# populationgenomics/cuKING

Hardware: AMD Instinct MI355X
Metric: sample-pairs/s (all-pairs KING) (higher is better)
Workload: dtype fp4 products, f32 accumulate (exact integers)

## Files before the change

cuking_amd/csrc/king_abi.hip:

```cpp
#include <hip/hip_runtime.h>

#include <algorithm>
#include <cstdio>
#include <cstdlib>
#include <cstring>
#include <vector>

#include "king_common.h"
#include "king_host.h"
#include "king_kin_summary.h"

using namespace cuking;

namespace {

#define HIP_TRY(expr)                                                      \
  do {                                                                     \
    const hipError_t _e = (expr);                                          \
    if (_e != hipSuccess) {                                                \
      (void)hipGetLastError();  \
      return cuking_fail(_e == hipErrorOutOfMemory ? CUKING_ERR_OUT_OF_MEMORY     \
                                            : CUKING_ERR_DEVICE,           \
                  "%s failed: %s", #expr, hipGetErrorString(_e));          \
    }                                                                      \
// ... 68 lines not shown
  struct StreamScratch {
    hipStream_t stream;
    uint32_t *split = nullptr;
    uint8_t *filter = nullptr;
    uint64_t filter_tiles = 0;
  };
  std::vector<StreamScratch> scratch;
  unsigned long long filter_totals_retired[kNumTotals] = {};
  uint32_t filter_quadrant_cap = kFilterQuadrantCap;
  uint32_t filter_cand_cap = kFilterCandCap;
  uint32_t filter_split_min_steps = 8;
  int filter_check0 = 1, filter_check1 = 1, filter_check_emit = (int)kCheckEmitCap;
  int filter_rotate = 1;
  uint32_t filter_rotate_min_steps = 128;
  uint32_t filter_rotate_min_tiles = 2048;
  int filter_sort = 1;
  bool filter_lazy_codes = true;
  void *sort_temp = nullptr;
  size_t sort_temp_bytes = 0;

  void *synth_tables = nullptr;
  size_t synth_tables_bytes = 0;
  hipStream_t synth_stream = nullptr;
  hipEvent_t synth_done = nullptr;

  struct Prepared {
    bool valid = false;
    cuking_submatrix sm = {0, 0, 0, 0};
    uint32_t words_per_sample = 0;
    int variant = -1;
// ... 179 lines not shown
         kin_threshold > 0.f && kin_threshold < 0.5f;
}

LaunchSwitches launch_switches(const cuking_ctx *ctx, uint32_t words_per_sample, bool full,
                               float kin_threshold) {
  LaunchSwitches sw;
  sw.xcd_swizzle = (uint32_t)ctx->xcd_swizzle;
  sw.dyn_tail_tiles = ctx->dyn_tail_tiles;
  sw.check0 = (uint32_t)ctx->filter_check0;
  sw.check1 = (uint32_t)ctx->filter_check1;
  sw.check_emit = (uint32_t)ctx->filter_check_emit;
  sw.rotate = (uint32_t)ctx->filter_rotate;
  sw.rotate_min_tiles = ctx->filter_rotate_min_tiles;
  sw.split_min_steps = ctx->filter_split_min_steps;
  sw.filter_runs = filter_runs(ctx, words_per_sample, full, kin_threshold);
  return sw;
}

struct Outputs {
  uint32_t max_results;
  cuking_result *results;
  uint32_t *result_index, *result_overflow;
  cuking_counts *counts;
  float *kin;
  uint64_t kin_ld;
  uint32_t kin_flags;
  uint64_t *sum_hist, *sum_best;
  cuking_kin_bins sum_bins;
  uint32_t *rel_counts;
  uint32_t rel_num;
// ... 32 lines not shown
  if (out.rel_counts != nullptr) {
    a.rel_num = out.rel_num;
    for (uint32_t t = 0; t < out.rel_num; ++t) a.rel_thr[t] = out.rel_thr[t];
  }
  a.rect_row_stride = 1;
  a.bits = d_bit_sets;
  a.words_per_sample = words_per_sample;
  a.split_wgs = ctx->split_wgs;
  if (plan_variant(ctx, words_per_sample).layout == kLayoutNibbleStats) {
    a.perm = plane_perm(ctx->planes, geo);
    if (!ctx->prepared.codes) a.codes_ready = plane_flags(ctx->planes, geo);
  }
  cuking_ctx::StreamScratch *e;
  const cuking_status st = scratch_for(ctx, stream, block_tiles, &e);
  if (st != CUKING_OK || e == nullptr) return st;
  if (uses_split_slab(ctx)) {
    a.split_counters = e->split;
    a.split_scratch = e->split + mfma_split_counter_bytes(ctx->split_wgs) / sizeof(uint32_t);
  }
  if (!uses_filter_scratch(ctx)) return CUKING_OK;
  uint8_t *base = e->filter;
  const FilterScratchLayout l = filter_scratch_layout(e->filter_tiles);
  a.sample_stats = plane_stats(ctx->planes, geo);
  a.t2 = plane_t2(ctx->planes, geo);
  a.prefix_u = plane_prefix_u(ctx->planes, geo);
  a.cohort_sums = plane_cohort_sums(ctx->planes, geo);
  a.filter_ctrl = reinterpret_cast<uint32_t *>(base);
  a.filter_totals = reinterpret_cast<unsigned long long *>(base + l.totals);
  a.fsplit_tickets = reinterpret_cast<uint32_t *>(base + l.tickets);
  a.tile_done = base + l.tile_done;
  a.cand_list = reinterpret_cast<uint2 *>(base + l.cand);
  a.cand_cap = ctx->filter_cand_cap < l.cand_entries ? ctx->filter_cand_cap : l.cand_entries;
  a.quadrant_cap = ctx->filter_quadrant_cap;
  a.dense_list = reinterpret_cast<uint2 *>(base + l.dense);
  a.dense_cap = l.chunk_tiles * 4;
  a.fsplit_slabs = ctx->split_wgs != 0 ? reinterpret_cast<float4 *>(base + l.slabs) : nullptr;
  a.rotate_min_steps = ctx->filter_rotate_min_steps;
  a.check_steps = plane_check_steps(ctx->planes, geo);
  return CUKING_OK;
}

hipError_t launch_planned(const cuking_ctx *ctx, uint32_t words_per_sample, bool full,
                          TiledArgs a, const LaunchSwitches &sw, uint64_t num_tiles,
                          hipStream_t stream) {
  const int kv = effective_variant(ctx, words_per_sample);
  if (tiled_variant(kv).tile != tiled_variant(ctx->variant).tile) {
    if (tiled_variant(kv).tile * 2 != tiled_variant(ctx->variant).tile) return hipErrorInvalidValue;
    to_quadrants(&a, &num_tiles);
  }
  return launch_tiled(kv, full, a, sw, num_tiles, stream);
}

// ... 312 lines not shown
    {"filter_sort", 0, 2, "filter_sort outside [0, 2]", 0, kInvalidatesLayout,
     CTX_FIELD(filter_sort)},
    {"filter_lazy_codes", 0, 1, "filter_lazy_codes outside [0, 1]", 0, kInvalidatesLayout,
     CTX_FIELD(filter_lazy_codes)},
    {"filter_check0", 0, 2, "filter_check0 outside [0, 2]", 0, 0, CTX_FIELD(filter_check0)},
    {"filter_check1", 0, 1 + kNumCheckShares, "filter_check1 outside {0, 1, 3 .. %u}",
     1 + kNumCheckShares, 0, CTX_FIELD(filter_check1), 2},
    {"filter_check_emit", 0, 255, "filter_check_emit outside [0, 255]", 0, 0,
     CTX_FIELD(filter_check_emit)},
    {"filter_rotate", 0, 2 + kNumPhases, "filter_rotate outside [0, %u]", 2 + kNumPhases, 0,
     CTX_FIELD(filter_rotate)},
    {"filter_rotate_min_steps", 1, 1 << 20, "filter_rotate_min_steps outside [1, 2^20]", 0, 0,
     CTX_FIELD(filter_rotate_min_steps)},
    {"filter_rotate_min_tiles", 0, 1 << 30, "filter_rotate_min_tiles outside [0, 2^30]", 0, 0,
     CTX_FIELD(filter_rotate_min_tiles)},
    {"filter_quadrant_cap", 0, 16384, "filter_quadrant_cap outside [0, 16384]", 0, 0,
     CTX_FIELD(filter_quadrant_cap)},
    {"filter_cand_cap", 0, kFilterCandCap, "filter_cand_cap outside [0, %u]", kFilterCandCap, 0,
     CTX_FIELD(filter_cand_cap)},
    {"filter_split_min_steps", 1, 4096, "filter_split_min_steps outside [1, 4096]", 0, 0,
     CTX_FIELD(filter_split_min_steps)},
    {"max_launch_blocks", 0, INT64_MAX, "negative block cap", 0, 0,
     [](const cuking_ctx *) -> int64_t { return (int64_t)max_blocks_override(); },
     [](cuking_ctx *, int64_t v) { set_max_blocks_per_launch((uint64_t)v); }},
    {"filter_check_min_steps", 4, 1 << 20, "filter_check_min_steps outside [4, 2^20]", 0,
     kInvalidatesLayout,
     [](const cuking_ctx *) -> int64_t { return filter_check_min_steps(); },
     [](cuking_ctx *, int64_t v) { set_filter_check_min_steps((uint32_t)v); }},
};
#undef CTX_FIELD
// ... 930 lines not shown
```

cuking_amd/csrc/king_common.h:

```cpp
#ifndef CUKING_AMD_KING_COMMON_H_
#define CUKING_AMD_KING_COMMON_H_

#include <hip/hip_runtime.h>
#include <stdint.h>

#include "cuking_amd.h"
#include "king_launch_plan.h"
#include "king_submatrix.h"

namespace cuking {

constexpr uint32_t kLayoutWord = 0;
constexpr uint32_t kLayoutQuad = 1;
constexpr uint32_t kLayoutNibble = 2;
constexpr uint32_t kLayoutNibbleStats = 3;

struct PlaneGeometry {
  uint32_t num_rows, num_cols;
  uint32_t rows_padded, cols_padded;
  uint32_t col_base;
  uint32_t s_stride;
  uint32_t k_words;
  uint32_t diag;
};
// ... 87 lines not shown
  const uint32_t *gate;
  uint32_t gate_count;
  const uint8_t *skip_tiles;
  uint64_t skip_base;
  const uint32_t *perm;
  uint32_t *codes_ready;
  float *dense_kin;
  uint64_t kin_ld;
  uint32_t kin_diag;
  unsigned long long *sum_hist, *sum_best;
  float sum_lo, sum_scale;
  uint32_t sum_bins;
  uint32_t *rel_counts;
  uint32_t rel_num;
  float rel_thr[CUKING_REL_THRESHOLDS_MAX];
};

constexpr uint32_t kCheckEmitCap = 64;
constexpr uint32_t kNumCheckShares = 8;
constexpr uint32_t kCheckShares64[kNumCheckShares] = {8, 50, 53, 56, 58, 60, 61, 62};
constexpr uint32_t kNumPhases = 128;
constexpr uint32_t kPhasesPerShare = kNumPhases / 64;
constexpr uint32_t kNumCum = kNumPhases - 1;
__host__ __device__ inline uint32_t phase_step(uint32_t all_steps, uint32_t x) {
  return (uint32_t)((uint64_t)all_steps * x / kNumPhases);
}
__host__ __device__ inline uint32_t check_step_of(uint32_t all_steps, uint32_t k,
                                                  uint32_t min_steps = 64) {
  if (all_steps < min_steps) return 0;
  return phase_step(all_steps, kCheckShares64[k] * kPhasesPerShare);
}
constexpr uint32_t kFilterSplitSlabs = 256;
constexpr size_t kFilterSlabBytes = 256 * 256 * sizeof(float);
constexpr size_t kFilterTicketBytes = kFilterSplitSlabs * sizeof(uint32_t);
__host__ __device__ inline size_t plane_bytes(const PlaneGeometry &g,
                                              uint32_t layout) {
  const size_t base = (size_t)g.k_words * g.s_stride * (layout == kLayoutQuad ? 8 : 16);
  if (layout == kLayoutNibble) return base + base / 4;
  if (layout == kLayoutNibbleStats)
    return base + base / 4 + base / 2 + (size_t)g.s_stride * sizeof(float2) +
// ... 34 lines not shown
static_assert(4ull * kMfmaN4MaxSites <= (1ull << 24), "filter kernel: exact float sums");
constexpr int kMfmaN4Stages = 5;
constexpr uint32_t kMfmaN4LdsBytes = kMfmaN4Stages * 2 * 2 * 4 * 128 * 16;
static_assert(kMfmaN4LdsBytes <= 160 * 1024, "LDS of one CU");
constexpr int kMfmaFilterVariant = 7;
constexpr uint32_t kFilterTile = 256;
constexpr uint32_t kFilterLdsBytes = 5 * 2 * 2 * 2 * 256 * 16;
static_assert(kFilterLdsBytes <= 160 * 1024, "LDS of one CU");
constexpr uint32_t kFilterChunkTiles = 1u << 17;
constexpr uint32_t kFilterCandCap = 1u << 25;
constexpr uint32_t kFilterQuadrantCap = 384;
constexpr size_t kFilterCtrlBytes = 256;
constexpr uint32_t kCtrlCand = 0, kCtrlDense = 1, kCtrlDyn = 2, kCtrlFinished = 3,
                   kCtrlLeft = 4, kCtrlAllLeave = 5, kCtrlGate = 6;
constexpr uint32_t kCtrlStepTicks = 8, kCtrlPos = 16, kPosSlots = 16;
constexpr size_t kCtrlChunkBytes = (kCtrlPos + 8 * kPosSlots * 2) * 4;
constexpr uint32_t kTotalCand = 0, kTotalDense = 1, kTotalEarly = 2, kTotalRotated = 3;
constexpr uint32_t kNumTotals = 4;
__host__ __device__ inline const uint32_t *plane_check_steps(const uint4 *planes,
                                                             const PlaneGeometry &g) {
  return reinterpret_cast<const uint32_t *>(plane_cohort_sums(planes, g) + 8);
}
__host__ __device__ inline uint32_t *plane_flags(const uint4 *planes, const PlaneGeometry &g) {
  return const_cast<uint32_t *>(plane_check_steps(planes, g)) + 16;
}
__host__ __device__ inline uint32_t *plane_perm(const uint4 *planes, const PlaneGeometry &g) {
  return plane_flags(planes, g) + 16;
}
__host__ __device__ inline float2 *plane_tmp_stats(const uint4 *planes, const PlaneGeometry &g) {
  return reinterpret_cast<float2 *>(plane_perm(planes, g) + g.s_stride);
}
// ... 32 lines not shown
constexpr uint32_t kMfmaLdsBytes = kMfmaStages * 2 * 2 * 2 * 128 * 16;
constexpr uint32_t kMfmaParkBytes = 4 * 64 * 64 * 4;
static_assert(kMfmaLdsBytes + kMfmaParkBytes <= 160 * 1024, "LDS of one CU");
const TiledVariant &tiled_variant(int v);
hipError_t launch_tiled(int variant, bool full, const TiledArgs &args, const LaunchSwitches &sw,
                        uint64_t num_tiles, hipStream_t stream);
hipError_t launch_mfma(bool full, bool nibble, const TiledArgs &args, const LaunchSwitches &sw,
                       uint64_t num_tiles, uint32_t lds_bytes, hipStream_t stream);
hipError_t launch_mfma_kin(bool nibble, const TiledArgs &args, const LaunchSwitches &sw,
                           uint64_t num_tiles, hipStream_t stream);
hipError_t launch_mfma_summary(bool nibble, const TiledArgs &args, const LaunchSwitches &sw,
                               uint64_t num_tiles, hipStream_t stream);
hipError_t launch_kin_mirror(float *d_kin, uint64_t ld, uint32_t n, hipStream_t stream);
hipError_t launch_mfma_list(const TiledArgs &args, const uint2 *list, const uint32_t *count,
                            uint32_t cap, uint32_t grid, hipStream_t stream);
hipError_t launch_mfma_gated(const TiledArgs &args, uint64_t num_units, const uint32_t *gate,
                             const uint8_t *skip_tiles, uint64_t skip_base, uint32_t grid,
                             hipStream_t stream);
hipError_t launch_filter(const TiledArgs &args, const LaunchSwitches &sw, uint64_t num_tiles,
                         hipStream_t stream);
inline void to_quadrants(TiledArgs *a, uint64_t *num_units) {
  a->quad = 1;
  a->tile_begin *= 4;
  *num_units *= 4;
}
hipError_t launch_sample_stats(const uint64_t *d_bit_sets, uint32_t words_per_sample,
                               const PlaneGeometry &geo, uint4 *d_planes, uint32_t s_begin,
                               uint32_t s_end, hipStream_t stream);
void set_filter_check_min_steps(uint32_t steps);
uint32_t filter_check_min_steps();
size_t sort_temp_bytes_for(uint32_t n);
hipError_t launch_sample_order(const PlaneGeometry &geo, uint32_t words_per_sample,
                               uint4 *d_planes, uint32_t s_begin, uint32_t s_end, bool sort,
                               void *sort_temp, size_t sort_temp_bytes, hipStream_t stream);
hipError_t launch_prepare_nibbles(bool codes, bool t2, const uint64_t *d_bit_sets,
                                  uint32_t words_per_sample, const PlaneGeometry &geo,
                                  uint4 *d_planes, const uint32_t *perm, uint32_t s_tile_begin,
                                  uint32_t s_tile_end, const uint32_t *gate,
                                  const uint32_t *ready, hipStream_t stream);
hipError_t launch_mark_codes_ready(const uint32_t *gate, uint32_t *ready, hipStream_t stream);
size_t mfma_split_scratch_bytes(uint32_t wgs);
size_t mfma_split_counter_bytes(uint32_t wgs);

void set_max_blocks_per_launch(uint64_t blocks);
uint64_t max_blocks_override();

hipError_t launch_prepare_planes(uint32_t layout, const uint64_t *d_bit_sets,
                                 uint32_t words_per_sample,
                                 const PlaneGeometry &geo, uint4 *d_planes,
                                 uint32_t s_tile_begin, uint32_t s_tile_end,
                                 hipStream_t stream);

hipError_t launch_stream(const cuking_submatrix &sm, uint32_t words_per_sample,
                         const uint64_t *d_bit_sets, float kin_threshold,
                         uint32_t max_results, cuking_result *d_results,
                         uint32_t *d_result_index, uint32_t *d_result_overflow,
                         cuking_counts *d_dense_counts, float *d_dense_kin, uint64_t kin_ld,
// ... 29 lines not shown
```

cuking_amd/csrc/king_device.h:

```cpp
#ifndef CUKING_AMD_KING_DEVICE_H_
#define CUKING_AMD_KING_DEVICE_H_

#include <hip/hip_runtime.h>

#include <atomic>

#include "king_common.h"

namespace cuking {

typedef __attribute__((address_space(3))) void *lds_void_ptr;
typedef const __attribute__((address_space(1))) void *global_void_ptr;

template <typename T>
__device__ __forceinline__ T relaxed_load(const T *p) {
  return __hip_atomic_load(p, __ATOMIC_RELAXED, __HIP_MEMORY_SCOPE_AGENT);
}
template <typename T, typename V>
__device__ __forceinline__ void relaxed_store(T *p, V v) {
  __hip_atomic_store(p, (T)v, __ATOMIC_RELAXED, __HIP_MEMORY_SCOPE_AGENT);
}
template <typename T, typename V>
__device__ __forceinline__ T relaxed_add(T *p, V v) {
  return __hip_atomic_fetch_add(p, (T)v, __ATOMIC_RELAXED, __HIP_MEMORY_SCOPE_AGENT);
// ... 5 lines not shown
  uint32_t lane, wave;
  uint32_t wy, wx;
  uint32_t g, lr;
};
__device__ __forceinline__ Lanes lanes_of_thread() {
  const uint32_t lane = threadIdx.x & 63;
  const uint32_t wave = __builtin_amdgcn_readfirstlane(threadIdx.x >> 6);
  return Lanes{lane, wave, wave >> 1, wave & 1, lane >> 5, lane & 31};
}

__device__ __forceinline__ uint32_t c_row(int r, uint32_t g) { return (r & 3) + 8 * (r >> 2) + 4 * g; }

__device__ __forceinline__ uint32_t xcd_patch_tile(uint32_t wg) {
  const uint32_t x = wg & 7, j = wg >> 3;
  return (((j >> 5) * 8 + x) << 5) + (j & 31);
}

__device__ __forceinline__ float king_kinship(uint32_t het_i, uint32_t het_j,
                                              uint32_t both_het,
                                              uint32_t opposing_hom) {
  const uint32_t min_hets = het_i < het_j ? het_i : het_j;
  const float num = 2.f * (float)both_het - 4.f * (float)opposing_hom -
                    (float)het_i - (float)het_j;
  const float den = 4.f * (float)min_hets;
  return 0.5f + num / den;
}

__device__ __forceinline__ void emit_result(uint32_t i, uint32_t j, float kin,
                                            uint32_t ibs0, uint32_t ibs1,
                                            uint32_t ibs2, uint32_t max_results,
// ... 292 lines not shown
```

cuking_amd/csrc/king_filter.hip:

```cpp
#include <hip/hip_runtime.h>
#include <stdio.h>

#include <atomic>
#include <stdlib.h>

#include "king_common.h"
#include "king_device.h"
#include "king_kin_summary.h"

#pragma clang diagnostic ignored "-Winline-asm"

namespace cuking {

namespace {

typedef int v8i __attribute__((ext_vector_type(8)));
typedef float v16f __attribute__((ext_vector_type(16)));

constexpr int kT = (int)kFilterTile;
constexpr int kUnits = 2;
constexpr int kStages = 5;
constexpr int kSliceU4 = kT;
constexpr int kStageU4 = 2 * 2 * kUnits * kSliceU4;
constexpr int kStageReqs = 4 * kUnits;
// ... 211 lines not shown
struct CheckPlan {
  uint32_t chk0, chk1;
  uint32_t share1;
  uint32_t phase;
  uint32_t k0;
  uint32_t wrap;
  uint32_t start_abs;
};
__device__ __forceinline__ CheckPlan plan_checks(const TiledArgs &a, const Tile &t,
                                                 const uint32_t xcd_pos, const uint32_t all_steps,
                                                 const uint32_t num_steps) {
  uint32_t chk0 = 0, chk1 = 0, entry1 = 0, share1 = 0;
  uint32_t phase = 0, k0 = 0, wrap = 0, start_abs = 0;
  if (!t.split && a.check_steps != nullptr && a.tile_done != nullptr) {
    if (a.rotate != 0 && all_steps >= a.rotate_min_steps) {
      uint32_t base = 0;
      if (a.rotate == 1) {
        const uint32_t r = xcd_pos % all_steps;
        base = xcd_pos - r;
        phase = (r * kNumPhases + all_steps / 2) / all_steps;
        if (phase >= kNumPhases) {
          phase = 0;
          base += all_steps;
        }
      } else if (a.rotate == 2) {
        phase = (t.bid * 37u + 11u) & (kNumPhases - 1);
      } else {
        phase = (a.rotate - 3u) & (kNumPhases - 1);
      }
      k0 = phase_step(all_steps, phase);
      start_abs = base + k0;
      wrap = k0 != 0 ? all_steps - k0 : 0u;
    }
    float kappa = -1.f, mean, sigma;
    if (bound_level(a.cohort_sums, 256.f * (float)all_steps, &mean, &sigma))
      kappa = mean + 4.6f * sigma + 0.003f;
    auto steps_of = [&](uint32_t share) {
      const uint32_t hi = phase + share * kPhasesPerShare;
      return hi <= kNumPhases ? phase_step(all_steps, hi) - k0
                              : (all_steps - k0) + phase_step(all_steps, hi - kNumPhases);
    };
    if ((a.check0 == 2 || (a.check0 == 1 && kappa > 0.7f * a.kin_threshold)) &&
        a.check_steps[0] != 0)
      chk0 = steps_of(kCheckShares64[0]);
    const uint32_t sw1 = a.check1 & 0xFFu;
    if (sw1 >= 2) {
      entry1 = sw1 - 2;
// ... 723 lines not shown
    if (a.codes_ready != nullptr) {
      e = launch_prepare_nibbles(true, false, a.bits, a.words_per_sample, a.geo,
                                 const_cast<uint4 *>(a.planes), a.perm, 0, 0xFFFFFFFFu,
                                 a.filter_ctrl, a.codes_ready, stream);
      if (e != hipSuccess) return e;
      e = launch_mark_codes_ready(a.filter_ctrl, a.codes_ready, stream);
      if (e != hipSuccess) return e;
    }
    e = launch_mfma_list(chunk, args.dense_list, args.filter_ctrl + kCtrlDense, args.dense_cap,
                         wgs, stream);
    if (e != hipSuccess) return e;
    if (checks) {
      TiledArgs f = chunk;
      uint64_t units = p.n;
      to_quadrants(&f, &units);
      e = launch_mfma_gated(f, units, args.filter_ctrl + kCtrlGate, args.tile_done,
                            chunk.tile_begin, wgs, stream);
      if (e != hipSuccess) return e;
    }
    done += p.n;
  }
  return hipSuccess;
}

}
```

cuking_amd/csrc/king_launch_plan.h:

```cpp
#ifndef CUKING_AMD_KING_LAUNCH_PLAN_H_
#define CUKING_AMD_KING_LAUNCH_PLAN_H_

#include <stdint.h>

namespace cuking {

struct LaunchSwitches {
  uint32_t xcd_swizzle, dyn_tail_tiles;
  uint32_t check0, check1, check_emit, rotate, rotate_min_tiles, split_min_steps;
  bool filter_runs;
};

struct WholeShape {
  uint64_t tiles;
  uint32_t launch_tiles, xcd_chunk, dyn_tiles, dyn_wgs;
  uint64_t grid;
};

inline WholeShape whole_shape(uint64_t want, uint64_t cap, uint32_t xcd_swizzle, uint64_t dyn_min,
                              uint64_t dyn_floor) {
  const bool xcd_order = xcd_swizzle != 0 && cap >= 64;
  if (xcd_order) cap &= ~7ull;
  uint64_t n = want < cap ? want : cap;
  WholeShape s = {};
  uint64_t dyn = 0, dyn_wgs = 0;
// ... 28 lines not shown
constexpr uint64_t kMfmaDynFloor = 512;
constexpr uint64_t kFilterDynFloor = 288;
inline uint64_t filter_dyn_min(uint32_t dyn_tail_tiles) {
  return dyn_tail_tiles == 0 ? 0 : dyn_tail_tiles < 4 ? 1 : dyn_tail_tiles / 4;
}

inline WholeShape split_shape(uint32_t split_whole, uint32_t wgs, uint32_t xcd_swizzle) {
  WholeShape s = {};
  s.tiles = split_whole;
  s.xcd_chunk = xcd_swizzle == 2 && split_whole != 0 && split_whole % 256 == 0;
  s.launch_tiles = split_whole;
  s.dyn_tiles = wgs;
  s.dyn_wgs = wgs + wgs / 2;
  s.grid = (uint64_t)split_whole + s.dyn_wgs;
  return s;
}

struct MfmaPlan {
  uint64_t first;
  uint32_t split_whole, split_tiles;
};
inline MfmaPlan mfma_plan(uint64_t num_tiles, uint32_t wgs, uint32_t tile_steps, uint64_t cap) {
  constexpr uint64_t kSplitRounds = 64;
  uint32_t rest = 0;
  if (wgs != 0 && num_tiles < kSplitRounds * wgs) {
    rest = num_tiles < 2ull * wgs ? (uint32_t)num_tiles : (uint32_t)(num_tiles % wgs);
    if ((uint64_t)rest * tile_steps < 8ull * wgs) rest = 0;
  }
  if (rest == 0) return {num_tiles, 0, 0};
  const uint64_t head = num_tiles - rest;
// ... 52 lines not shown
```

cuking_amd/csrc/king_mfma.hip:

```cpp
#include <hip/hip_runtime.h>

#include "king_common.h"
#include "king_device.h"
#include "king_kin_summary.h"

#pragma clang diagnostic ignored "-Winline-asm"

namespace cuking {

namespace {

typedef int v8i __attribute__((ext_vector_type(8)));
typedef float v16f __attribute__((ext_vector_type(16)));

constexpr int kTile = 128;
constexpr int kStageU4 = 2 * 2 * 2 * kTile;
constexpr int kPiecesPerWave = 4;
constexpr int kStagesPaired = 10;
constexpr uint32_t kMfmaSummaryLdsBytes = 2 * kTile * 8 + (CUKING_KIN_BINS_MAX + 3) * 4;
static_assert(kMfmaSummaryLdsBytes <= kStagesPaired * kStageU4 * 16 &&
                  kMfmaSummaryLdsBytes <= kMfmaN4LdsBytes,
              "the summary's LDS fits the stages of either lean form");

constexpr int kA = 0x08;
// ... 543 lines not shown
    }
  CUKING_MMA16(1, Y)
  CUKING_MMA4(1, Y)
  CUKING_EXPAND(Y, As, Bs, m1)
  CUKING_MMA16(2, X)
  CUKING_MMA4(2, X)
  CUKING_MMA16(3, Y)
  CUKING_MMA4(3, Y)
#undef CUKING_LOAD_RAW
#undef CUKING_EXPAND
#undef CUKING_MMA1
#undef CUKING_MMA16
#undef CUKING_MMA4
}

template <bool FULL>
__device__ __forceinline__ void four_product_loop(const TiledArgs &a, const Segment &s,
                                                  const Lanes &l, const NibbleMasks &m,
                                                  uint4 *const lds, v16f (&acc)[2][2][kNQ],
                                                  v16f (&hh5)[2][2]) {
  constexpr bool HH5 = FULL;
  constexpr int NSTAGE = stages_of(FULL, true);
  const uint32_t wave = l.wave, g = l.g, lr = l.lr, wr = l.wy * 64, wc = l.wx * 64;
  const uint32_t s_stride = a.geo.s_stride, k_first = s.k_first, num_steps = s.num_steps;
  const uint32_t m1 = m.m1, m2 = m.m2;
  uint32_t lane16 = l.lane * 16;
  const uint32_t dma_side = wave >> 1, dma_kg = wave & 1;
  const uint4 *g_rows = a.planes + (uint64_t)s.tr * kTile;
  const uint4 *g_cols = a.planes + a.geo.col_base + (uint64_t)s.tc * kTile;
  constexpr int kSliceU4 = kTile;
  constexpr int kStageN4 = 2 * 2 * 4 * kSliceU4;
  uint32_t mT;
  asm volatile("s_mov_b32 %0, 0xcccccccc" : "=s"(mT));
  const uint32_t mH = m1, mD = m2;
  const uint4 *const g_wave4 = (dma_side ? g_cols : g_rows) +
                               (uint64_t)(8 * k_first + 4 * dma_kg) * s_stride;
  const uint32_t l_wave4 = (uint32_t)(uintptr_t)(lds_void_ptr)(
      lds + ((dma_side * 2 + dma_kg) * 4) * kSliceU4);
  struct N4Addr { const uint4 *src; uint32_t dst; };
  auto n4_addr = [&](uint32_t step, uint32_t buf) {
    N4Addr pa;
    if (step >= num_steps) step = num_steps - 1;
    pa.src = g_wave4 + (uint64_t)step * 8 * s_stride;
    pa.dst = l_wave4 + buf * (kStageN4 * 16);
    asm volatile("" : "+s"(pa.src), "+s"(pa.dst));
    return pa;
  };
  const uint32_t kstep_bytes = 8 * s_stride * 16;
  auto n4_next = [&](const N4Addr &cur, uint32_t step, uint32_t buf) {
    N4Addr pa;
    const uint32_t adv = step < num_steps ? kstep_bytes : 0u;
    pa.src = reinterpret_cast<const uint4 *>(reinterpret_cast<const char *>(cur.src) + adv);
    pa.dst = l_wave4 + buf * (kStageN4 * 16);
    asm volatile("" : "+s"(pa.src), "+s"(pa.dst));
    return pa;
  };
  auto n4_issue = [&](const N4Addr &pa, int c, int half) {
    const uint4 *src = pa.src + (uint64_t)c * s_stride;
    const uint32_t dst = pa.dst + c * (kSliceU4 * 16);
    if (half) CUKING_LDS_DMA(dst, src, " offset:1024");
    else CUKING_LDS_DMA(dst, src, "");
  };
  auto n4_sync = [&]() {
    __builtin_amdgcn_s_waitcnt(vmcnt_imm(2 * 8 + 4));
    __syncthreads();
  };
  auto n4_prologue = [&]() {
// ... 103 lines not shown
  uint32_t buf = 0;
  N4Addr pa = n4_addr(NSTAGE - 1, NSTAGE - 1);
#define N4_KSTEP                                                               \
  {                                                                            \
    const uint32_t nbuf = buf == NSTAGE - 1 ? 0 : buf + 1;                     \
    N4Addr pa_next;                                                            \
    N4_SLICE(0, 1, buf, 2, false, 0)                                           \
    N4_SLICE(1, 0, buf, 3, false, 1)                                           \
    N4_SLICE(0, 1, nbuf, 0, true, 2)                                           \
    N4_SLICE(1, 0, nbuf, 1, false, 3)                                          \
    pa = pa_next;                                                              \
    buf = nbuf;                                                                \
    ++step;                                                                    \
  }
  uint32_t step = 0;
  while (step + 3 < num_steps) {
    N4_KSTEP
    N4_KSTEP
    N4_KSTEP
    N4_KSTEP
  }
  while (step < num_steps) N4_KSTEP
#undef N4_KSTEP
#undef N4_READ
#undef N4_PIN4
#undef N4_PINF
#undef N4_PIN_RAW_A
#undef N4_PIN_RAW_B
#undef N4_PIN_A
#undef N4_PIN_B
#undef N4_BUILD_A
#undef N4_BUILD_B
#undef N4_MMA
#undef N4_DMA_GROUP
#undef N4_READ_GROUP
#undef N4_LAST_GROUP
#undef N4_SLICE
// ... 384 lines not shown
constexpr int kRecords = 0, kKinMatrix = 1, kKinSummary = 2, kRelCounts = 3;
template <bool FULL, bool SPLIT, bool N4 = false, int KIN = kRecords>
__global__ __launch_bounds__(256, 1) void king_mfma_kernel(const TiledArgs a) {
  static_assert(KIN == kRecords || !FULL, "the dense-kinship forms are lean ones");
  extern __shared__ uint4 lds[];
  Work work;
  if (!take_work<SPLIT>(a, lds, &work)) return;
  const Lanes l = lanes_of_thread();
  const NibbleMasks m = nibble_masks();
  uint32_t lane16 = l.lane * 16;
  Segment s;
  while (next_segment<SPLIT>(a, &work, &s)) {
    v16f hh5[2][2];
    v16f acc[2][2][kNQ];
    if constexpr (FULL) hom_hom_pass<N4>(a, s, l, m, lds, hh5);
    if constexpr (N4) four_product_loop<FULL>(a, s, l, m, lds, acc, hh5);
    else five_product_loop<FULL>(a, s, l, m, lds, lane16, acc);
    __builtin_amdgcn_s_waitcnt(0x0F70);
    if (SPLIT) __syncthreads();

    float4 *const park = FULL && !N4 ? park_slots(lds, l) : nullptr;
    if (SPLIT && s.num_steps != tile_steps_of(a) &&
        !reduce_parts<FULL, N4>(a, work.piece, s, l, lds, park, acc, hh5))
      continue;

    if constexpr (FULL) {
      if (a.dense_counts == nullptr) emit_full_records<N4>(a, s, l, park, acc, hh5);
      else store_counts<N4>(a, s, l, park, acc, hh5);
    } else if constexpr (KIN == kKinMatrix) {
      store_kin<N4>(a, s, l, acc);
    } else if constexpr (KIN == kKinSummary) {
      summarise_kin<N4>(a, s, l, lds, acc);
    } else if constexpr (KIN == kRelCounts) {
      count_relatives<N4>(a, s, l, acc);
    } else {
      lean_decide<N4>(a, s, l, acc);
    }
    if (SPLIT) __syncthreads();
  }
}

void set_shape(TiledArgs *a, const WholeShape &s) {
  a->launch_tiles = s.launch_tiles;
  a->xcd_chunk = s.xcd_chunk;
  a->dyn_tiles = s.dyn_tiles;
  a->dyn_wgs = s.dyn_wgs;
}

template <bool FULL, bool SPLIT, bool N4 = false, int KIN = kRecords>
hipError_t launch_shape(const TiledArgs &args, const LaunchSwitches &sw, uint64_t num_blocks,
                        uint32_t lds_bytes, hipStream_t stream) {
  constexpr auto kernel = king_mfma_kernel<FULL, SPLIT, N4, KIN>;
  if (N4) lds_bytes = kMfmaN4LdsBytes;
  else if (FULL) lds_bytes += kMfmaParkBytes;
  else lds_bytes = kStagesPaired * kStageU4 * sizeof(uint4);
  hipError_t e = allow_dynamic_lds<kernel>(lds_bytes);
  if (e != hipSuccess) return e;
  TiledArgs a = args;
  if (SPLIT) {
    const WholeShape s = split_shape(args.split_whole, args.split_wgs, sw.xcd_swizzle);
    set_shape(&a, s);
    kernel<<<dim3((uint32_t)s.grid), dim3(256), lds_bytes, stream>>>(a);
    return hipGetLastError();
  }
  const uint64_t dyn_min = args.split_counters != nullptr ? sw.dyn_tail_tiles : 0;
  const uint64_t cap = max_blocks_per_launch(256);
  for (uint64_t done = 0; done < num_blocks;) {
    const WholeShape s = whole_shape(num_blocks - done, cap, sw.xcd_swizzle, dyn_min, kMfmaDynFloor);
    a.tile_begin = args.tile_begin + done;
    set_shape(&a, s);
    kernel<<<dim3((uint32_t)s.grid), dim3(256), lds_bytes, stream>>>(a);
    e = hipGetLastError();
    if (e != hipSuccess) return e;
    done += s.tiles;
  }
  return hipSuccess;
}

}

size_t mfma_split_scratch_bytes(uint32_t wgs) {
  return split_counter_bytes(wgs) + (size_t)wgs * 2 * (4 * 4 * 5 * 16 * 64) * sizeof(float);
}
size_t mfma_split_counter_bytes(uint32_t wgs) { return split_counter_bytes(wgs); }

namespace {
hipError_t launch_form(bool full, bool split, bool nibble, int kin, const TiledArgs &a,
                       const LaunchSwitches &sw, uint64_t blocks, uint32_t lds_bytes,
                       hipStream_t stream) {
  if (kin < kRecords || kin > kRelCounts || (kin != kRecords && full)) return hipErrorInvalidValue;
  using Launch = hipError_t (*)(const TiledArgs &, const LaunchSwitches &, uint64_t, uint32_t,
                                hipStream_t);
  static constexpr Launch kForms[4][2][2][2] = {
      {{{launch_shape<false, false, false>, launch_shape<true, false, false>},
        {launch_shape<false, true, false>, launch_shape<true, true, false>}},
       {{launch_shape<false, false, true>, launch_shape<true, false, true>},
        {launch_shape<false, true, true>, launch_shape<true, true, true>}}},
      {{{launch_shape<false, false, false, kKinMatrix>, nullptr},
        {launch_shape<false, true, false, kKinMatrix>, nullptr}},
// ... 29 lines not shown
  if (grid == 0) return hipErrorInvalidValue;
  return lean_form_of(a) == kRelCounts ? launch_strided_form<kRelCounts>(a, grid, stream)
                                       : launch_strided_form<kRecords>(a, grid, stream);
}
}

hipError_t launch_mfma_list(const TiledArgs &args, const uint2 *list, const uint32_t *count,
                            uint32_t cap, uint32_t grid, hipStream_t stream) {
  if (list == nullptr) return hipErrorInvalidValue;
  TiledArgs a = args;
  a.tile_begin = 0;
  a.rect_rows = 0;
  a.tile_list = list;
  a.tile_list_count = count;
  a.tile_list_cap = cap;
  return launch_strided(a, grid, stream);
}

hipError_t launch_mfma_gated(const TiledArgs &args, uint64_t num_units, const uint32_t *gate,
                             const uint8_t *skip_tiles, uint64_t skip_base, uint32_t grid,
                             hipStream_t stream) {
  if (gate == nullptr || num_units > 0xFFFFFFFFull) return hipErrorInvalidValue;
  TiledArgs a = args;
  a.gate = gate;
  a.gate_count = (uint32_t)num_units;
  a.skip_tiles = skip_tiles;
  a.skip_base = skip_base;
  return launch_strided(a, grid, stream);
}

namespace {
hipError_t launch_planned_form(bool full, bool nibble, int kin, const TiledArgs &args,
                               const LaunchSwitches &sw, uint64_t num_tiles, uint32_t lds_bytes,
                               hipStream_t stream) {
  if ((uint64_t)args.geo.k_words * 32 > (nibble ? kMfmaN4MaxSites : kMfmaMaxSites))
    return hipErrorInvalidValue;
  const MfmaPlan p = mfma_plan(num_tiles, args.split_scratch != nullptr ? args.split_wgs : 0,
                               args.geo.k_words / 8, max_blocks_per_launch(256));
  hipError_t e = launch_form(full, false, nibble, kin, args, sw, p.first, lds_bytes, stream);
  if (e != hipSuccess || p.split_tiles == 0) return e;
  TiledArgs a = args;
  a.tile_begin = args.tile_begin + p.first;
// ... 63 lines not shown
```

Baseline: 39.59 billion.

## Rotate k-loop start phase in MFMA kernel using per-XCD published positions

Lets the nibble MFMA product loop start its k-steps at a rotated phase and wrap around, so concurrently running workgroups on the same XCD stream different slices of the sample bit data. This is meant to spread memory traffic and improve L2/MALL reuse. With rotate mode 1, each workgroup reads timestamped progress records from per-XCD position slots, extrapolates where its neighbours are now, picks its phase from that, and publishes its own progress every 16 steps through lane-0 stores. The cost is extra global writes and reads, a chunked loop with a wrap branch, and reliance on realtime-clock extrapolation.

Result: no change. 39.55 billion, median of 2 (-0.1%).

```diff
diff --git a/cuking_amd/csrc/king_abi.hip b/cuking_amd/csrc/king_abi.hip
--- a/cuking_amd/csrc/king_abi.hip
+++ b/cuking_amd/csrc/king_abi.hip
@@ -106,6 +106,7 @@
   int filter_rotate = 1;
   uint32_t filter_rotate_min_steps = 128;
   uint32_t filter_rotate_min_tiles = 2048;
+  int mfma_rotate = 1;
   int filter_sort = 1;
   bool filter_lazy_codes = true;
   void *sort_temp = nullptr;
@@ -315,6 +316,7 @@
   sw.rotate_min_tiles = ctx->filter_rotate_min_tiles;
   sw.split_min_steps = ctx->filter_split_min_steps;
   sw.filter_runs = filter_runs(ctx, words_per_sample, full, kin_threshold);
+  sw.mfma_rotate = (uint32_t)ctx->mfma_rotate;
   return sw;
 }
 
@@ -377,9 +379,12 @@
   cuking_ctx::StreamScratch *e;
   const cuking_status st = scratch_for(ctx, stream, block_tiles, &e);
   if (st != CUKING_OK || e == nullptr) return st;
+  a.rotate_min_steps = ctx->filter_rotate_min_steps;
   if (uses_split_slab(ctx)) {
     a.split_counters = e->split;
     a.split_scratch = e->split + mfma_split_counter_bytes(ctx->split_wgs) / sizeof(uint32_t);
+    a.mfma_pos = reinterpret_cast<uint4 *>(reinterpret_cast<uint8_t *>(e->split) +
+                                           mfma_split_pos_offset(ctx->split_wgs));
   }
   if (!uses_filter_scratch(ctx)) return CUKING_OK;
   uint8_t *base = e->filter;
@@ -398,7 +403,6 @@
   a.dense_list = reinterpret_cast<uint2 *>(base + l.dense);
   a.dense_cap = l.chunk_tiles * 4;
   a.fsplit_slabs = ctx->split_wgs != 0 ? reinterpret_cast<float4 *>(base + l.slabs) : nullptr;
-  a.rotate_min_steps = ctx->filter_rotate_min_steps;
   a.check_steps = plane_check_steps(ctx->planes, geo);
   return CUKING_OK;
 }
@@ -741,6 +745,7 @@
      CTX_FIELD(filter_rotate_min_steps)},
     {"filter_rotate_min_tiles", 0, 1 << 30, "filter_rotate_min_tiles outside [0, 2^30]", 0, 0,
      CTX_FIELD(filter_rotate_min_tiles)},
+    {"mfma_rotate", 0, 2, "mfma_rotate outside [0, 2]", 0, 0, CTX_FIELD(mfma_rotate)},
     {"filter_quadrant_cap", 0, 16384, "filter_quadrant_cap outside [0, 16384]", 0, 0,
      CTX_FIELD(filter_quadrant_cap)},
     {"filter_cand_cap", 0, kFilterCandCap, "filter_cand_cap outside [0, %u]", kFilterCandCap, 0,
diff --git a/cuking_amd/csrc/king_common.h b/cuking_amd/csrc/king_common.h
--- a/cuking_amd/csrc/king_common.h
+++ b/cuking_amd/csrc/king_common.h
@@ -125,6 +125,8 @@
   uint32_t *rel_counts;
   uint32_t rel_num;
   float rel_thr[CUKING_REL_THRESHOLDS_MAX];
+  uint4 *mfma_pos;
+  uint32_t mfma_epoch;
 };
 
 constexpr uint32_t kCheckEmitCap = 64;
@@ -135,6 +137,28 @@
 constexpr uint32_t kNumCum = kNumPhases - 1;
 __host__ __device__ inline uint32_t phase_step(uint32_t all_steps, uint32_t x) {
   return (uint32_t)((uint64_t)all_steps * x / kNumPhases);
+}
+struct Rotation {
+  uint32_t phase, k0, wrap, start_abs;
+};
+__host__ __device__ inline Rotation rotation_of(uint32_t rotate, uint32_t bid, uint32_t xcd_pos,
+                                                uint32_t all_steps) {
+  uint32_t phase, base = 0;
+  if (rotate == 1) {
+    const uint32_t r = xcd_pos % all_steps;
+    base = xcd_pos - r;
+    phase = (r * kNumPhases + all_steps / 2) / all_steps;
+    if (phase >= kNumPhases) {
+      phase = 0;
+      base += all_steps;
+    }
+  } else if (rotate == 2) {
+    phase = (bid * 37u + 11u) & (kNumPhases - 1);
+  } else {
+    phase = (rotate - 3u) & (kNumPhases - 1);
+  }
+  const uint32_t k0 = phase_step(all_steps, phase);
+  return Rotation{phase, k0, k0 != 0 ? all_steps - k0 : 0u, base + k0};
 }
 __host__ __device__ inline uint32_t check_step_of(uint32_t all_steps, uint32_t k,
                                                   uint32_t min_steps = 64) {
@@ -199,7 +223,10 @@
 constexpr uint32_t kCtrlCand = 0, kCtrlDense = 1, kCtrlDyn = 2, kCtrlFinished = 3,
                    kCtrlLeft = 4, kCtrlAllLeave = 5, kCtrlGate = 6;
 constexpr uint32_t kCtrlStepTicks = 8, kCtrlPos = 16, kPosSlots = 16;
-constexpr size_t kCtrlChunkBytes = (kCtrlPos + 8 * kPosSlots * 2) * 4;
+constexpr size_t kMfmaPosBytes = 8 * kPosSlots * 16;
+constexpr uint32_t kCtrlMfmaPos = kCtrlPos + 8 * kPosSlots * 2;
+static_assert(kCtrlMfmaPos % 4 == 0, "16-byte slots");
+constexpr size_t kCtrlChunkBytes = kCtrlMfmaPos * 4 + kMfmaPosBytes;
 constexpr uint32_t kTotalCand = 0, kTotalDense = 1, kTotalEarly = 2, kTotalRotated = 3;
 constexpr uint32_t kNumTotals = 4;
 __host__ __device__ inline const uint32_t *plane_check_steps(const uint4 *planes,
@@ -262,9 +289,9 @@
 hipError_t launch_kin_mirror(float *d_kin, uint64_t ld, uint32_t n, hipStream_t stream);
 hipError_t launch_mfma_list(const TiledArgs &args, const uint2 *list, const uint32_t *count,
                             uint32_t cap, uint32_t grid, hipStream_t stream);
-hipError_t launch_mfma_gated(const TiledArgs &args, uint64_t num_units, const uint32_t *gate,
-                             const uint8_t *skip_tiles, uint64_t skip_base, uint32_t grid,
-                             hipStream_t stream);
+hipError_t launch_mfma_gated(const TiledArgs &args, const LaunchSwitches &sw, uint64_t num_units,
+                             const uint32_t *gate, const uint8_t *skip_tiles, uint64_t skip_base,
+                             uint32_t grid, hipStream_t stream);
 hipError_t launch_filter(const TiledArgs &args, const LaunchSwitches &sw, uint64_t num_tiles,
                          hipStream_t stream);
 inline void to_quadrants(TiledArgs *a, uint64_t *num_units) {
@@ -289,6 +316,7 @@
 hipError_t launch_mark_codes_ready(const uint32_t *gate, uint32_t *ready, hipStream_t stream);
 size_t mfma_split_scratch_bytes(uint32_t wgs);
 size_t mfma_split_counter_bytes(uint32_t wgs);
+size_t mfma_split_pos_offset(uint32_t wgs);
 
 void set_max_blocks_per_launch(uint64_t blocks);
 uint64_t max_blocks_override();
diff --git a/cuking_amd/csrc/king_device.h b/cuking_amd/csrc/king_device.h
--- a/cuking_amd/csrc/king_device.h
+++ b/cuking_amd/csrc/king_device.h
@@ -43,6 +43,23 @@
 __device__ __forceinline__ uint32_t xcd_patch_tile(uint32_t wg) {
   const uint32_t x = wg & 7, j = wg >> 3;
   return (((j >> 5) * 8 + x) << 5) + (j & 31);
+}
+
+__device__ __forceinline__ uint32_t position_now(uint32_t pos, uint32_t when, uint32_t rate_steps,
+                                                 uint32_t rate_ticks, uint32_t window) {
+  const uint32_t ago = (uint32_t)__builtin_amdgcn_s_memrealtime() - when;
+  if (rate_ticks != 0 && ago < window) pos += ago * rate_steps / rate_ticks;
+  return pos;
+}
+__device__ __forceinline__ void store_lane0_b64(void *p, unsigned long long v, uint32_t zero) {
+  unsigned long long save;
+  asm volatile("s_mov_b64 %0, exec\n\t"
+               "s_mov_b64 exec, 1\n\t"
+               "global_store_dwordx2 %1, %2, %3\n\t"
+               "s_mov_b64 exec, %0"
+               : "=&s"(save)
+               : "v"(zero), "v"(v), "s"(p)
+               : "memory");
 }
 
 __device__ __forceinline__ float king_kinship(uint32_t het_i, uint32_t het_j,
diff --git a/cuking_amd/csrc/king_filter.hip b/cuking_amd/csrc/king_filter.hip
--- a/cuking_amd/csrc/king_filter.hip
+++ b/cuking_amd/csrc/king_filter.hip
@@ -249,23 +249,11 @@
   uint32_t phase = 0, k0 = 0, wrap = 0, start_abs = 0;
   if (!t.split && a.check_steps != nullptr && a.tile_done != nullptr) {
     if (a.rotate != 0 && all_steps >= a.rotate_min_steps) {
-      uint32_t base = 0;
-      if (a.rotate == 1) {
-        const uint32_t r = xcd_pos % all_steps;
-        base = xcd_pos - r;
-        phase = (r * kNumPhases + all_steps / 2) / all_steps;
-        if (phase >= kNumPhases) {
-          phase = 0;
-          base += all_steps;
-        }
-      } else if (a.rotate == 2) {
-        phase = (t.bid * 37u + 11u) & (kNumPhases - 1);
-      } else {
-        phase = (a.rotate - 3u) & (kNumPhases - 1);
-      }
-      k0 = phase_step(all_steps, phase);
-      start_abs = base + k0;
-      wrap = k0 != 0 ? all_steps - k0 : 0u;
+      const Rotation r = rotation_of(a.rotate, t.bid, xcd_pos, all_steps);
+      phase = r.phase;
+      k0 = r.k0;
+      start_abs = r.start_abs;
+      wrap = r.wrap;
     }
     float kappa = -1.f, mean, sigma;
     if (bound_level(a.cohort_sums, 256.f * (float)all_steps, &mean, &sigma))
@@ -1019,7 +1007,8 @@
       TiledArgs f = chunk;
       uint64_t units = p.n;
       to_quadrants(&f, &units);
-      e = launch_mfma_gated(f, units, args.filter_ctrl + kCtrlGate, args.tile_done,
+      f.mfma_pos = reinterpret_cast<uint4 *>(args.filter_ctrl + kCtrlMfmaPos);
+      e = launch_mfma_gated(f, sw, units, args.filter_ctrl + kCtrlGate, args.tile_done,
                             chunk.tile_begin, wgs, stream);
       if (e != hipSuccess) return e;
     }
diff --git a/cuking_amd/csrc/king_launch_plan.h b/cuking_amd/csrc/king_launch_plan.h
--- a/cuking_amd/csrc/king_launch_plan.h
+++ b/cuking_amd/csrc/king_launch_plan.h
@@ -9,6 +9,7 @@
   uint32_t xcd_swizzle, dyn_tail_tiles;
   uint32_t check0, check1, check_emit, rotate, rotate_min_tiles, split_min_steps;
   bool filter_runs;
+  uint32_t mfma_rotate;
 };
 
 struct WholeShape {
@@ -67,6 +68,13 @@
   s.dyn_wgs = wgs + wgs / 2;
   s.grid = (uint64_t)split_whole + s.dyn_wgs;
   return s;
+}
+
+inline uint32_t mfma_rotate(const LaunchSwitches &sw, uint64_t tiles, bool has_slots,
+                            bool persistent) {
+  if (sw.mfma_rotate == 0 || sw.rotate == 0 || (persistent && sw.mfma_rotate < 2)) return 0;
+  if (sw.rotate >= 2) return sw.rotate;
+  return has_slots && tiles >= sw.rotate_min_tiles ? 1u : 0u;
 }
 
 struct MfmaPlan {
diff --git a/cuking_amd/csrc/king_mfma.hip b/cuking_amd/csrc/king_mfma.hip
--- a/cuking_amd/csrc/king_mfma.hip
+++ b/cuking_amd/csrc/king_mfma.hip
@@ -1,4 +1,6 @@
 #include <hip/hip_runtime.h>
+
+#include <atomic>
 
 #include "king_common.h"
 #include "king_device.h"
@@ -581,11 +583,70 @@
 #undef CUKING_MMA4
 }
 
-template <bool FULL>
+constexpr uint32_t kPublishSteps = 16;
+constexpr uint32_t kNoWrap = 0xFFFFFFFFu;
+struct Turn {
+  uint32_t k0;
+  uint32_t wrap;
+  uint4 *slot;
+  uint32_t start_abs;
+  uint32_t tag;
+  uint32_t t_start;
+};
+__device__ __forceinline__ uint32_t xcd_position(const TiledArgs &a, uint4 *const lds) {
+  uint32_t *const words = reinterpret_cast<uint32_t *>(lds);
+  if (threadIdx.x < kPosSlots) {
+    const unsigned long long *slot = reinterpret_cast<const unsigned long long *>(
+        a.mfma_pos + (blockIdx.x & 7) * kPosSlots + threadIdx.x);
+    const unsigned long long said = relaxed_load(slot), rate = relaxed_load(slot + 1);
+    const uint32_t tagged = (uint32_t)(said >> 32);
+    words[threadIdx.x] = (tagged >> 24) == a.mfma_epoch
+                             ? position_now(tagged & 0xFFFFFFu, (uint32_t)said, (uint32_t)rate,
+                                            (uint32_t)(rate >> 32), 65536u)
+                             : 0u;
+  }
+  __syncthreads();
+  uint32_t pos = 0;
+#pragma unroll
+  for (uint32_t k = 0; k < kPosSlots; ++k) pos = max(pos, words[k]);
+  pos = __builtin_amdgcn_readfirstlane(pos);
+  __syncthreads();
+  return pos;
+}
+template <bool SPLIT>
+__device__ __forceinline__ Turn begin_turn(const TiledArgs &a, const Segment &s, uint4 *const lds) {
+  Turn t = {0, kNoWrap, nullptr, 0, 0, 0};
+  const uint32_t all_steps = tile_steps_of(a);
+  if (SPLIT || a.rotate == 0 || all_steps < a.rotate_min_steps) return t;
+  const uint32_t pos = a.rotate == 1 ? xcd_position(a, lds) : 0u;
+  const Rotation r = rotation_of(a.rotate, s.tile, pos, all_steps);
+  auto sgpr = [](uint32_t v) { return (uint32_t)__builtin_amdgcn_readfirstlane(v); };
+  t.k0 = sgpr(r.k0);
+  t.wrap = sgpr(r.wrap != 0 ? r.wrap : kNoWrap);
+  if (a.rotate == 1) {
+    t.slot = a.mfma_pos + (blockIdx.x & 7) * kPosSlots + ((blockIdx.x >> 3) & (kPosSlots - 1));
+    t.start_abs = sgpr(r.start_abs);
+    t.tag = a.mfma_epoch << 24;
+    t.t_start = (uint32_t)__builtin_amdgcn_s_memrealtime();
+  }
+  return t;
+}
+__device__ __forceinline__ void publish_turn(const Turn &t, uint32_t wave, uint32_t steps,
+                                             uint32_t zero) {
+  if (t.slot != nullptr && wave == 0) {
+    const uint32_t now = (uint32_t)__builtin_amdgcn_s_memrealtime();
+    const uint32_t tagged = t.tag | ((t.start_abs + steps) & 0xFFFFFFu);
+    unsigned long long *const w = reinterpret_cast<unsigned long long *>(t.slot);
+    store_lane0_b64(w, ((unsigned long long)tagged << 32) | now, zero);
+    store_lane0_b64(w + 1, ((unsigned long long)(now - t.t_start) << 32) | steps, zero);
+  }
+}
+
+template <bool FULL, bool TURNS>
 __device__ __forceinline__ void four_product_loop(const TiledArgs &a, const Segment &s,
                                                   const Lanes &l, const NibbleMasks &m,
-                                                  uint4 *const lds, v16f (&acc)[2][2][kNQ],
-                                                  v16f (&hh5)[2][2]) {
+                                                  const Turn &turn, uint4 *const lds,
+                                                  v16f (&acc)[2][2][kNQ], v16f (&hh5)[2][2]) {
   constexpr bool HH5 = FULL;
   constexpr int NSTAGE = stages_of(FULL, true);
   const uint32_t wave = l.wave, g = l.g, lr = l.lr, wr = l.wy * 64, wc = l.wx * 64;
@@ -601,23 +662,28 @@
   asm volatile("s_mov_b32 %0, 0xcccccccc" : "=s"(mT));
   const uint32_t mH = m1, mD = m2;
   const uint4 *const g_wave4 = (dma_side ? g_cols : g_rows) +
-                               (uint64_t)(8 * k_first + 4 * dma_kg) * s_stride;
+                               (uint64_t)(8 * (k_first + turn.k0) + 4 * dma_kg) * s_stride;
+  const uint32_t wrap = turn.wrap, all_steps = tile_steps_of(a);
   const uint32_t l_wave4 = (uint32_t)(uintptr_t)(lds_void_ptr)(
       lds + ((dma_side * 2 + dma_kg) * 4) * kSliceU4);
   struct N4Addr { const uint4 *src; uint32_t dst; };
+  const uint32_t kstep_bytes = 8 * s_stride * 16;
   auto n4_addr = [&](uint32_t step, uint32_t buf) {
     N4Addr pa;
     if (step >= num_steps) step = num_steps - 1;
-    pa.src = g_wave4 + (uint64_t)step * 8 * s_stride;
+    const int32_t rel = (int32_t)step - (int32_t)(TURNS && step >= wrap ? all_steps : 0u);
+    pa.src = reinterpret_cast<const uint4 *>(reinterpret_cast<const char *>(g_wave4) +
+                                             (int64_t)rel * (int64_t)kstep_bytes);
     pa.dst = l_wave4 + buf * (kStageN4 * 16);
     asm volatile("" : "+s"(pa.src), "+s"(pa.dst));
     return pa;
   };
-  const uint32_t kstep_bytes = 8 * s_stride * 16;
   auto n4_next = [&](const N4Addr &cur, uint32_t step, uint32_t buf) {
     N4Addr pa;
     const uint32_t adv = step < num_steps ? kstep_bytes : 0u;
-    pa.src = reinterpret_cast<const uint4 *>(reinterpret_cast<const char *>(cur.src) + adv);
+    const uint32_t back = TURNS && step == wrap ? all_steps : 0u;
+    pa.src = reinterpret_cast<const uint4 *>(reinterpret_cast<const char *>(cur.src) + adv -
+                                             (uint64_t)back * kstep_bytes);
     pa.dst = l_wave4 + buf * (kStageN4 * 16);
     asm volatile("" : "+s"(pa.src), "+s"(pa.dst));
     return pa;
@@ -751,13 +817,27 @@
     ++step;                                                                    \
   }
   uint32_t step = 0;
-  while (step + 3 < num_steps) {
-    N4_KSTEP
-    N4_KSTEP
-    N4_KSTEP
-    N4_KSTEP
-  }
-  while (step < num_steps) N4_KSTEP
+#pragma nounroll
+  while (true) {
+    uint32_t lim = num_steps;
+    if constexpr (TURNS) {
+      if (turn.slot != nullptr) {
+        lim = step + kPublishSteps;
+        if (wrap > step && wrap < lim) lim = wrap;
+        if (lim > num_steps) lim = num_steps;
+      }
+      lim = __builtin_amdgcn_readfirstlane(lim);
+    }
+    while (step + 3 < lim) {
+      N4_KSTEP
+      N4_KSTEP
+      N4_KSTEP
+      N4_KSTEP
+    }
+    while (step < lim) N4_KSTEP
+    if constexpr (TURNS) publish_turn(turn, wave, step, lane16);
+    if (!TURNS || step >= num_steps) break;
+  }
 #undef N4_KSTEP
 #undef N4_READ
 #undef N4_PIN4
@@ -1172,7 +1252,10 @@
     v16f hh5[2][2];
     v16f acc[2][2][kNQ];
     if constexpr (FULL) hom_hom_pass<N4>(a, s, l, m, lds, hh5);
-    if constexpr (N4) four_product_loop<FULL>(a, s, l, m, lds, acc, hh5);
+    if constexpr (N4) {
+      const Turn turn = begin_turn<SPLIT>(a, s, lds);
+      four_product_loop<FULL, !SPLIT>(a, s, l, m, turn, lds, acc, hh5);
+    }
     else five_product_loop<FULL>(a, s, l, m, lds, lane16, acc);
     __builtin_amdgcn_s_waitcnt(0x0F70);
     if (SPLIT) __syncthreads();
@@ -1196,6 +1279,15 @@
     }
     if (SPLIT) __syncthreads();
   }
+}
+
+uint32_t next_epoch() {
+  static std::atomic<uint32_t> launches{0};
+  return 1 + launches.fetch_add(1, std::memory_order_relaxed) % 255;
+}
+void set_rotation(TiledArgs *a, const LaunchSwitches &sw, uint64_t tiles, bool persistent) {
+  a->rotate = mfma_rotate(sw, tiles, a->mfma_pos != nullptr, persistent);
+  a->mfma_epoch = a->rotate == 1 ? next_epoch() : 0;
 }
 
 void set_shape(TiledArgs *a, const WholeShape &s) {
@@ -1218,6 +1310,7 @@
   if (SPLIT) {
     const WholeShape s = split_shape(args.split_whole, args.split_wgs, sw.xcd_swizzle);
     set_shape(&a, s);
+    a.rotate = 0;
     kernel<<<dim3((uint32_t)s.grid), dim3(256), lds_bytes, stream>>>(a);
     return hipGetLastError();
   }
@@ -1227,6 +1320,7 @@
     const WholeShape s = whole_shape(num_blocks - done, cap, sw.xcd_swizzle, dyn_min, kMfmaDynFloor);
     a.tile_begin = args.tile_begin + done;
     set_shape(&a, s);
+    if (N4) set_rotation(&a, sw, s.tiles, false);
     kernel<<<dim3((uint32_t)s.grid), dim3(256), lds_bytes, stream>>>(a);
     e = hipGetLastError();
     if (e != hipSuccess) return e;
@@ -1238,9 +1332,10 @@
 }
 
 size_t mfma_split_scratch_bytes(uint32_t wgs) {
-  return split_counter_bytes(wgs) + (size_t)wgs * 2 * (4 * 4 * 5 * 16 * 64) * sizeof(float);
-}
-size_t mfma_split_counter_bytes(uint32_t wgs) { return split_counter_bytes(wgs); }
+  return mfma_split_counter_bytes(wgs) + (size_t)wgs * 2 * (4 * 4 * 5 * 16 * 64) * sizeof(float);
+}
+size_t mfma_split_counter_bytes(uint32_t wgs) { return split_counter_bytes(wgs) + kMfmaPosBytes; }
+size_t mfma_split_pos_offset(uint32_t wgs) { return split_counter_bytes(wgs); }
 
 namespace {
 hipError_t launch_form(bool full, bool split, bool nibble, int kin, const TiledArgs &a,
@@ -1300,18 +1395,20 @@
   a.tile_list = list;
   a.tile_list_count = count;
   a.tile_list_cap = cap;
+  a.rotate = 0;
   return launch_strided(a, grid, stream);
 }
 
-hipError_t launch_mfma_gated(const TiledArgs &args, uint64_t num_units, const uint32_t *gate,
-                             const uint8_t *skip_tiles, uint64_t skip_base, uint32_t grid,
-                             hipStream_t stream) {
+hipError_t launch_mfma_gated(const TiledArgs &args, const LaunchSwitches &sw, uint64_t num_units,
+                             const uint32_t *gate, const uint8_t *skip_tiles, uint64_t skip_base,
+                             uint32_t grid, hipStream_t stream) {
   if (gate == nullptr || num_units > 0xFFFFFFFFull) return hipErrorInvalidValue;
   TiledArgs a = args;
   a.gate = gate;
   a.gate_count = (uint32_t)num_units;
   a.skip_tiles = skip_tiles;
   a.skip_base = skip_base;
+  set_rotation(&a, sw, num_units, true);
   return launch_strided(a, grid, stream);
 }
 
```
